# Stalfoes/dqn_mgsc_zoo

Measured on AMD Instinct MI355X. Metric: learner grad-steps/sec at batch=32, 84×84×4 uint8, 1/2/4/8 MI355X, higher is better.
Workload: dtype f32

## Files before the change

dqn_mgsc_zoo_amd/_native.py:

```python

import ctypes
import glob
import hashlib
import os
import threading

_HERE = os.path.dirname(os.path.abspath(__file__))
LIB_PATH = os.environ.get('DQZ_LIB') or os.path.join(_HERE, 'libdqz.so')
HEADER_PATH = os.path.join(os.path.dirname(_HERE), 'include', 'dqz.h')

DQZ_OK = 0
ALGO_DQN = 0
ALGO_DOUBLE = 1
ALGO_PER = 2
NUM_LEAVES = 10
NUM_PHASES = 10
PHASE_NAMES = (
    'conv1_fwd', 'conv2_fwd', 'conv3_fwd', 'fc1_fwd', 'head', 'fc1_dx',
    'conv3_dx+conv2_dx+fc1_dw+conv3_dw+conv2_dw+conv1_dw', 'unused7',
    'unused8', 'update')
FRAME_H = 84
FRAME_W = 84
STACK = 4
FRAME_BYTES = FRAME_H * FRAME_W
# ... 209 lines not shown
        _int, [ctypes.POINTER(DqzLearnerConfig), _int, _vp,
               ctypes.POINTER(_vp)]),
    'dqz_c51_destroy': (_int, [_vp]),
    'dqz_c51_learner': (_int, [_vp, ctypes.POINTER(_vp)]),
    'dqz_c51_step': (
        _int,
        [_vp, ctypes.POINTER(DqzParams), ctypes.POINTER(DqzStore), _vp, _vp,
         _vp, _vp]),
    'dqz_c51_grad': (
        _int,
        [_vp, ctypes.POINTER(DqzParams), ctypes.POINTER(DqzStore), _vp, _vp,
         _vp]),
    'dqz_c51_outputs': (_int, [_vp, _vp, _vp, _vp, _vp, _vp, _vp]),
    'dqz_c51_debug': (_int, [_vp, _vp, _vp, _vp]),
    'dqz_c51_profile': (
        _int,
        [_vp, ctypes.POINTER(DqzParams), ctypes.POINTER(DqzStore), _vp, _vp,
         _int, ctypes.POINTER(ctypes.c_float), _vp]),
    'dqz_c51_forward': (_int, [_vp, _vp, _vp, _int, _vp, _vp]),
    'dqz_c51_forward_slots': (
        _int, [_vp, _vp, ctypes.POINTER(DqzStore), _vp, _int, _int, _vp, _vp]),
    'dqz_c51_act': (
        _int, [_vp, _vp, _vp, _int, ctypes.c_double, ctypes.c_uint64,
               ctypes.c_uint64, _vp, _vp]),
    'dqz_c51_debug_check': (_int, [_int, ctypes.c_uint]),
    'dqz_learner_grad': (
        _int,
        [_vp, ctypes.POINTER(DqzParams), ctypes.POINTER(DqzStore), _vp, _vp,
         _vp, _vp],
    ),
    'dqz_learner_outputs': (_int, [_vp, _vp, _vp, _vp, _vp]),
    'dqz_learner_sync_status': (_int, [_vp, _vp]),
    'dqz_learner_debug_stall': (_int, [_vp, _int, ctypes.c_uint]),
    'dqz_learner_debug_activations': (_int, [_vp, _int] + [_vp] * 10),
    'dqz_per_write_back': (_int, [_vp, _vp, _i64, _vp, ctypes.c_double, _vp, _vp]),
    'dqz_learner_profile': (
        _int,
        [_vp, ctypes.POINTER(DqzParams), ctypes.POINTER(DqzStore), _vp, _vp,
         _int, ctypes.POINTER(ctypes.c_float), _vp],
    ),
    'dqz_forward': (_int, [_vp, _vp, _vp, _int, _vp, _vp]),
    'dqz_forward_slots': (
        _int, [_vp, _vp, ctypes.POINTER(DqzStore), _vp, _int, _int, _vp, _vp]),
    'dqz_act': (
        _int, [_vp, _vp, _vp, _int, ctypes.c_double, ctypes.c_uint64,
               ctypes.c_uint64, _vp, _vp]),
    'dqz_store_put': (
        _int, [ctypes.POINTER(DqzStore), ctypes.POINTER(DqzTransitionPut), _vp,
               _vp]),
    'dqz_store_jumble': (
        _int, [ctypes.POINTER(DqzStore), ctypes.POINTER(DqzJumble), _vp]),
    'dqz_logits_census': (_int, [_vp, _vp, _vp, _i64, _i64, _vp, _vp]),
    'dqz_frame_plan_create': (_int, [_int, _int, _int, _int, ctypes.POINTER(_vp)]),
    'dqz_frame_plan_destroy': (_int, [_vp]),
    'dqz_atari_frame': (_int, [_vp, _vp, _int, _vp, _vp]),
    'dqz_sample_uniform': (
        _int, [_i64, _i64, _i64, _int, ctypes.c_uint64, _vp, _vp, _vp]),
    'dqz_gather_stacks': (
        _int, [ctypes.POINTER(DqzStore), _vp, _int, _int, _vp, _vp]),
    'dqz_target_copy': (_int, [_vp, _vp, _i64, _vp]),
    'dqz_logit_buffer_create': (_int, [_i64, _int, ctypes.POINTER(_vp)]),
    'dqz_logit_buffer_destroy': (_int, [_vp]),
    'dqz_logits_add': (_int, [_vp, _vp, _i64, _i64, _i64, _vp, _vp]),
    'dqz_logits_sample': (_int, [_vp, _vp, _vp, _int, _vp, _vp]),
    'dqz_logits_sample_slots': (
        _int, [_vp, _vp, ctypes.c_uint64, _vp, _vp, _int, _vp, _vp, _vp]),
# ... 130 lines not shown
```

dqn_mgsc_zoo_amd/csrc/bwd.hpp:

```cpp
#pragma once
#include "common.hpp"
#include "conv1.hpp"
#include "fwd.hpp"
#include "head.hpp"
#include "sampling.hpp"

namespace dqz {

struct Fc1BwdArgs {
  const float* dz1;
  const float* y3;
  float *th, *mu, *nu;
  int64_t w_off;
  Rms rms;
  int B;
  float* dy3;
  const float *w3, *w2;
  float *w3p, *w2p;
};

__device__ __forceinline__ int w3p_src(int i) {
  const int j = i & 3, kq = (i >> 2) & 3, n = (i >> 4) & 15, w = (i >> 8) & 3, r = i >> 10;
  const int tp = r % 9, nq = r / 9;
  return ((8 - tp) * C3CI + 16 * nq + n) * C3CO + 16 * w + 4 * j + kq;
// ... 217 lines not shown
    for (int tp = 0; tp < 9; ++tp) {
      const int off = (tp / 3) * C3W_RS + (tp % 3) * C3W_S;
      acc[tp] = mfma4(dr[kk], s_win[pb[kk] + off], acc[tp]);
    }
  float sb = 0.f;
#pragma unroll
  for (int kk = 0; kk < 13; ++kk) sb += dr[kk];
  float* slab = a.part + (int64_t)b * (C3KK + 1) * C3CO;
#pragma unroll
  for (int tp = 0; tp < 9; ++tp)
    *reinterpret_cast<f32x4*>(slab + (tp * C3CI + 16 * w + n) * C3CO + 16 * nq + 4 * kq) = acc[tp];
  if (w == 0) {
    sb += __shfl_xor(sb, 16, 64);
    sb += __shfl_xor(sb, 32, 64);
    if (kq == 0) slab[C3KK * C3CO + 16 * nq + n] = sb;
  }
}

constexpr int C2X_S = 66, C2X_RS = 756, C2X_WIN = 11 * C2X_RS;
constexpr int C2W_S = 40, C2W_RS = 808, C2W_WIN = 20 * C2W_RS;

struct Conv2BwdArgs {
  const float* dy2;
  const float* y1;
  const float* w2;
  const float* w2p;
  float* dy1;
  float* part;
  int B;
  Handoff sync;
  Handoff sync1;
};

template <bool WAIT, bool PUB = false>
__device__ __forceinline__ void conv2_bwd_dx(const Conv2BwdArgs& a, float* s_win, int b, int ph, int pw, int hh) {
  const int t = threadIdx.x, lane = t & 63, w = t >> 6;
  const int n = lane & 15, kq = lane >> 4;
  float wr[16];
  {
    const float4* wp =
        reinterpret_cast<const float4*>(a.w2p) + (((((ph * 2 + pw) * 2 + hh) * 4) * 4 + w) * 16 + n) * 4 + kq;
#pragma unroll
    for (int tp = 0; tp < 4; ++tp) {
      const float4 v = wp[tp * 256];
      wr[4 * tp] = v.x;
      wr[4 * tp + 1] = v.y;
      wr[4 * tp + 2] = v.z;
      wr[4 * tp + 3] = v.w;
    }
  }
  float4 ym4[2];
#pragma unroll
  for (int k = 0; k < 2; ++k) {
    const int q = min((t >> 2) + 64 * k, 99), ah = q / 10, cw = q % 10;
    ym4[k] = *reinterpret_cast<const float4*>(a.y1 + ((int64_t)b * C1M + (2 * ah + ph) * C1O + 2 * cw + pw) * C1CO +
                                              16 * hh + 4 * (t & 3));
  }
  const float4* src = reinterpret_cast<const float4*>(a.dy2 + (int64_t)b * (C2M * C2CO));
  constexpr int NW4 = 121 * 16;
  if constexpr (WAIT) a.sync.wait(b);
  float4 r[8];
#pragma unroll
  for (int q = 0; q < 8; ++q) {
    const int i = min(t + 256 * q, NW4 - 1);
    const int pix = i >> 4, oh = pix / 11 - 1, ow = pix % 11 - 1;
    const bool in = oh >= 0 && oh < C2O && ow >= 0 && ow < C2O;
    const int e = (in ? oh * C2O + ow : 0) * 16 + (i & 15);
    float4 v;
    if constexpr (WAIT)
      v = load_sc1_f4(src, C2M * C2CO * 4, e);
    else
      v = src[e];
    r[q] = in ? v : make_float4(0.f, 0.f, 0.f, 0.f);
  }
  __builtin_amdgcn_sched_barrier(0);
#pragma unroll
  for (int q = 0; q < 8; ++q) {
    const int i = t + 256 * q;
    if (i < NW4) {
      const int pix = i >> 4;
      float* d = s_win + (pix / 11) * C2X_RS + (pix % 11) * C2X_S + win64_ch((i & 15) * 4);
      d[0] = r[q].x;
      d[1] = r[q].y;
      d[2] = r[q].z;
      d[3] = r[q].w;
    }
  }
  __syncthreads();
  DQZ_STAMP(7, 1);
// ... 340 lines not shown
  d += dpp_f<0x140>(d);
  if ((t & 15) == 0) a.dy3[r] = ym > 0.f ? d : 0.f;
  if (a.w3p) {
    if (g < W3P_N) a.w3p[g] = v3;
    if (g < W2P_N) a.w2p[g] = v2;
  }
  DQZ_STAMP(5, 3);
}

#ifdef DQZ_STEP_TU
inline hipError_t launch_head_dx1(const HeadArgs& h, const Fc1BwdArgs& f, hipStream_t st) {
  if (h.S > 7 || h.Z < 1 || h.Z > 3 || h.B != 1) return hipErrorInvalidValue;
  const dim3 grid(FC1X1_BLOCKS), block(512);
  if (h.A <= 8) {
    if (h.Z <= 2)
      hipLaunchKernelGGL((head_dx1_kernel<8, 7, 2>), grid, block, 0, st, h, f);
    else
      hipLaunchKernelGGL((head_dx1_kernel<8, 7, 3>), grid, block, 0, st, h, f);
  } else {
    if (h.Z <= 2)
      hipLaunchKernelGGL((head_dx1_kernel<MAXA, 7, 2>), grid, block, 0, st, h, f);
    else
      hipLaunchKernelGGL((head_dx1_kernel<MAXA, 7, 3>), grid, block, 0, st, h, f);
  }
  return hipGetLastError();
}
#endif

DQZ_STEP_KERNEL __launch_bounds__(256) void fc1_dx_kernel(Fc1BwdArgs a) {
  __shared__ __attribute__((aligned(16))) float smem[FC1X_SMEM];
  fc1_dx_block(a, smem, blockIdx.x);
}

template <bool WB>
__global__ __launch_bounds__(256) __attribute__((amdgpu_waves_per_eu(4, 8))) void bwd_bc_kernel(
    Conv3BwdArgs c3, Fc1BwdArgs f1, Conv2BwdArgs c2, Conv1DwArgs c1, PerWbArgs wb) {
  constexpr int kW = C3X_WIN > FC1W_SMEM ? C3X_WIN : FC1W_SMEM;
  constexpr int kW2 = C2X_WIN > C3W_WIN ? C2X_WIN : C3W_WIN;
  constexpr int kW3 = C2V_WIN > C1H_SMEM ? C2V_WIN : C1H_SMEM;
  constexpr int kWA = kW > kW2 ? kW : kW2;
  constexpr int kSmem = kWA > kW3 ? kWA : kW3;
  static_assert(kSmem * 4 >= PWB_LDS_BYTES, "the write-back's LDS comes out of the backward's buffer");
  __shared__ __attribute__((aligned(16))) float smem[kSmem];
  const int B8 = (c3.B + 7) / 8 * 8;
  constexpr int NF = 4 * (FLAT / 16);
  int i = blockIdx.x;
  if constexpr (WB) {
    if (i < 8) {
      if (i == 0 && threadIdx.x < 64) per_write_back_wave(wb, reinterpret_cast<char*>(smem));
      return;
    }
    i -= 8;
  }
  if (i < 8 * B8) {
    const SampleJob sj = xcd_sample_job_at(i, 8, c3.B);
    if (!sj.valid) return;
    __builtin_amdgcn_s_setprio(3);
    DQZ_STAMP(6, 0);
    conv3_bwd_dx<true>(c3, smem, sj.s, sj.job & 3, sj.job >> 2);
    DQZ_STAMP(6, 3);
    return;
  }
  i -= 8 * B8;
  if (i < NF) {
    fc1_dw_body(f1, smem, i);
    return;
  }
  i -= NF;
  if (i < 8 * B8) {
    const SampleJob sj = xcd_sample_job_at(i, 8, c2.B);
    if (!sj.valid) return;
    __builtin_amdgcn_s_setprio(3);
    DQZ_STAMP(7, 0);
    conv2_bwd_dx<true, true>(c2, smem, sj.s, (sj.job & 3) >> 1, sj.job & 1, sj.job >> 2);
    DQZ_STAMP(7, 3);
    return;
  }
  i -= 8 * B8;
  if (i < 4 * B8) {
    const SampleJob sj = xcd_sample_job_at(i, 4, c3.B);
    if (!sj.valid) return;
    DQZ_STAMP(12, 0);
    conv3_bwd_dw(c3, smem, sj.s, sj.job);
    DQZ_STAMP(12, 3);
    return;
  }
  i -= 4 * B8;
  if (i < 8 * B8) {
    const SampleJob sj = xcd_sample_job_at(i, 8, c1.B);
    if (!sj.valid) return;
    __builtin_amdgcn_s_setprio(2);
    conv1_dw_half(c1, smem, sj.job >> 1, sj.job & 1, sj.s);
    return;
  }
  i -= 8 * B8;
  const SampleJob sj = xcd_sample_job_at(i, 8, c2.B);
  if (!sj.valid) return;
  DQZ_STAMP(13, 0);
  conv2_bwd_dw_split(c2, smem, sj.s, sj.job >> 1, sj.job & 1);
  DQZ_STAMP(13, 3);
}

}
```

dqn_mgsc_zoo_amd/csrc/conv1.hpp:

```cpp
#pragma once
#include "common.hpp"
#include "sampling.hpp"

namespace dqz {

struct Conv1Src {
  const uint8_t* frames;
  const int32_t* fidx;
  const int32_t* slots;
  const uint8_t* states;
  int fused;
  union {
    UniformDraw draw;
    SoftmaxDraw sm;
    PerSampleArgs per;
    SoftmaxDrawExact smx;
  };
  const int32_t* action = nullptr;
  const float* reward = nullptr;
  const float* discount = nullptr;
  float4* rec = nullptr;
  uint8_t* xout = nullptr;
};

// ... 212 lines not shown
    for (int e = 0; e < 4; ++e) {
      const float y = div255(sum[e]) + bb[e];
      v[e] = linear ? y : relu(y);
    }
    if constexpr (PUB) {
      store_sc1_f4(out, C1_POS * C1CO * 4, 16 * i, v);
    } else if (dot) {
      const f32x4 d = *reinterpret_cast<const f32x4*>(dyp + 4 * i);
      dacc += ((v[0] * d[0] + v[1] * d[1]) + (v[2] * d[2] + v[3] * d[3]));
    } else {
      *reinterpret_cast<f32x4*>(out + 4 * i) = v;
    }
  }
  if constexpr (PUB) a.pub.arrive(sj.s);
  if (!PUB && dot) {
    __syncthreads();
    const float r = block_sum256(dacc, smem);
    if (threadIdx.x == 0) a.dot.part[(int64_t)b * META_DOT_SLOTS + a.dot.slot0 + rb] = r;
  }
  DQZ_STAMP(0, 3);
}

struct Conv1DwArgs {
  Conv1Src src;
  int which, B;
  const float* dy1;
  float* part;
  Handoff sync1;
};

constexpr int C1H_TLD = 136;
constexpr int C1H_SMEM = (2 * C1_PLANE * 2 + 3 * C1CO * C1H_TLD * 2) / 4 + 16 * C1CO;

__device__ __forceinline__ void conv1_dw_half(const Conv1DwArgs& a, float* smem, int rb, int ch, int b) {
  DQZ_STAMP(8, 0);
  uint16_t* s_in = reinterpret_cast<uint16_t*>(smem);
  uint16_t* s_dt = s_in + 2 * C1_PLANE;
  float* s_bp = smem + (2 * C1_PLANE + 3 * C1CO * C1H_TLD) / 2;
  const int row0 = rb * C1S * C1_ROWS;
  constexpr int QPC = C1_PLANE / 16;
  const int slot = a.src.slots[b];
  const int32_t* fr = a.src.fidx + (int64_t)slot * 8 + a.which * 4 + 2 * ch;
  const int fa = fr[0], fb = fr[1];
  uint4 v = make_uint4(0u, 0u, 0u, 0u);
  const int tid = threadIdx.x;
  const int cl = tid / QPC, pj = tid % QPC;
  const int f = cl == 0 ? fa : fb;
  if (tid < 2 * QPC && f >= 0)
    v = reinterpret_cast<const uint4*>(a.src.frames + (int64_t)f * FB + row0 * FW)[pj];
  a.sync1.wait(b);
  const float* dyb = a.dy1 + ((int64_t)b * C1M + rb * C1_POS) * C1CO;
  const int co = tid & 31, c0 = tid >> 5;
  float dv[2][8];
#pragma unroll
  for (int it = 0; it < 2; ++it) {
    const int c = c0 + 8 * it, oh = c / 3, ow0 = 8 * (c % 3);
#pragma unroll
    for (int j = 0; j < 8; ++j)
      dv[it][j] = (c < 15 && ow0 + j < C1O)
                      ? load_sc1_f1(dyb, C1_POS * C1CO * 4, (oh * C1O + ow0 + j) * C1CO + co) : 0.f;
  }
  if (tid < 2 * QPC) store_bytes_as_bf16(s_in + cl * C1_PLANE + pj * 16, v);
#pragma unroll
  for (int it = 0; it < 2; ++it) {
    const int c = c0 + 8 * it;
    unsigned pk[3][4];
    float sb = 0.f;
#pragma unroll
    for (int j = 0; j < 8; j += 2) {
      unsigned h0, m0, l0, h1, m1, l1;
      split3_bf16(dv[it][j], h0, m0, l0);
      split3_bf16(dv[it][j + 1], h1, m1, l1);
      pk[0][j / 2] = h0 | (h1 << 16);
      pk[1][j / 2] = m0 | (m1 << 16);
      pk[2][j / 2] = l0 | (l1 << 16);
      sb += dv[it][j];
      sb += dv[it][j + 1];
    }
#pragma unroll
    for (int q = 0; q < 3; ++q)
      *reinterpret_cast<uint4*>(s_dt + (q * C1CO + co) * C1H_TLD + 8 * c) =
          make_uint4(pk[q][0], pk[q][1], pk[q][2], pk[q][3]);
// ... 9 lines not shown
    for (int c = 0; c < 15; ++c) sb += s_bp[c * C1CO + tid];
    part[C1KK * C1CO + tid] = sb;
  }
  const int kh = 2 * wave + (i >> 4), kw = (i >> 1) & 7, cp = i & 1;
  const uint16_t* pb = s_in + cp * C1_PLANE + kh * FW + kw;
  const uint16_t* pa = s_dt + i * C1H_TLD + 8 * h;
  f32x16 acc = {};
#pragma unroll
  for (int s = 0; s < 8; ++s) {
    constexpr int R = 4 * FW;
    const int o0 = (2 * s) / 3 * R + 32 * ((2 * s) % 3);
    const int o1 = 2 * s + 1 < 15 ? (2 * s + 1) / 3 * R + 32 * ((2 * s + 1) % 3) : 0;
    const uint16_t* px = pb + (h ? o1 : o0);
    unsigned xp[4];
#pragma unroll
    for (int j = 0; j < 8; j += 2) xp[j / 2] = (unsigned)px[4 * j] | ((unsigned)px[4 * j + 4] << 16);
    const bf16x8 xb = __builtin_bit_cast(bf16x8, make_uint4(xp[0], xp[1], xp[2], xp[3]));
#pragma unroll
    for (int q = 0; q < 3; ++q) {
      const bf16x8 dq = __builtin_bit_cast(bf16x8, *reinterpret_cast<const uint4*>(pa + q * C1CO * C1H_TLD + 16 * s));
      acc = __builtin_amdgcn_mfma_f32_32x32x16_bf16(dq, xb, acc, 0, 0, 0);
    }
  }
  {
    const int row = (2 * wave + (i >> 4)) * 32 + ((i >> 1) & 7) * 4 + 2 * ch + (i & 1);
#pragma unroll
    for (int q = 0; q < 4; ++q)
      *reinterpret_cast<f32x4*>(part + row * C1CO + 8 * q + 4 * h) =
          f32x4{div255(acc[4 * q]), div255(acc[4 * q + 1]), div255(acc[4 * q + 2]), div255(acc[4 * q + 3])};
  }
  DQZ_STAMP(8, 3);
}

}
```

dqn_mgsc_zoo_amd/csrc/learner_impl.hpp:

```cpp
#pragma once
#include <hip/hip_runtime.h>

#include <cstring>

#include "common.hpp"
#include "layout.hpp"
#include "conv1.hpp"
#include "fwd.hpp"
#include "head.hpp"
#include "bwd.hpp"
#include "sampling.hpp"

namespace dqz {

inline void param_layout(int A, int shared_bias, int64_t off[10], int64_t sz[10], int64_t* total) {
  const int64_t sizes[10] = {C1KK * C1CO, C1CO, C2KK * C2CO, C2CO, C3KK * C3CO, C3CO,
                             (int64_t)FLAT * HID, HID, (int64_t)HID * A, shared_bias ? 1 : A};
  int64_t o = 0;
  for (int i = 0; i < 10; ++i) {
    off[i] = o;
    sz[i] = sizes[i];
    o += (sizes[i] + 63) / 64 * 64;
  }
  *total = o;
}

}

struct dqz_learner {
  dqz_learner_config cfg;
  int Z, shared_bias;
  int64_t off[10], sz[10], total;
  int S_fc1, S2, S3;
  float *y1, *y2, *y3, *fc1p, *h1, *q, *dz1, *dy3, *dy2, *dy1, *p1, *p2, *p3, *td, *loss, *loss_part, *gq, *rec;
  float *w3p, *w2p;
  double* per_wb;
  int32_t* ga;
  int32_t* sync;
  unsigned spin_max = 1u << 24;
  void* block;
};

namespace dqz {

static_assert(Handoff::kStride == kWordStride, "layout.hpp's word stride is Handoff's");

inline SyncLayout sync_of(const dqz_learner* L) { return SyncLayout{L->cfg.batch}; }
inline Handoff handoff(const dqz_learner* L, const HandoffWords& w) {
  Handoff h{L->sync + w.cnt, L->sync + w.ack, L->sync + sync_of(L).err(), w.need, w.consumers};
  if (w.learner_spin) h.spin_max = L->spin_max;
  return h;
}

inline int check_store(const dqz_store* S) {
  if (!S || !S->frames || !S->fidx || !S->action || !S->reward || !S->discount)
    return fail(DQZ_ERR_INVALID, "store has a null buffer");
  if (S->capacity < 1) return fail(DQZ_ERR_INVALID, "store capacity must be positive");
  return DQZ_OK;
}

inline int device_view(const void* p, const void** out, const char* what) {
  hipPointerAttribute_t attr;
  if (hipPointerGetAttributes(&attr, p) != hipSuccess) {
    (void)hipGetLastError();
    return fail(DQZ_ERR_INVALID, "%s must be device memory or pinned host memory", what);
  }
  if (attr.type == hipMemoryTypeHost) {
    void* d = attr.devicePointer;
    if (!d && hipHostGetDevicePointer(&d, const_cast<void*>(p), 0) != hipSuccess) {
      (void)hipGetLastError();
      return fail(DQZ_ERR_INVALID, "%s: pinned host memory without a device mapping", what);
    }
    *out = d;
  } else if (attr.type == hipMemoryTypeDevice || attr.type == hipMemoryTypeManaged ||
             attr.type == hipMemoryTypeUnified) {
    *out = p;
  } else {
    return fail(DQZ_ERR_INVALID, "%s must be device memory or pinned host memory", what);
  }
  return DQZ_OK;
}

struct PhaseEvents {
  hipEvent_t e0, e1;
// ... 109 lines not shown
```

dqn_mgsc_zoo_amd/csrc/learner_step.hip:

```cpp
#define DQZ_STEP_TU 1
#include <hip/hip_runtime.h>

#include <cstdlib>
#include <cstring>

#include "learner_impl.hpp"

using namespace dqz;

static int g_attr_done = 0;

static int init_kernel_attrs() {
  if (g_attr_done) return DQZ_OK;
  const void* fwd_kernels[] = {(const void*)fwd_conv_kernel<0>, (const void*)fwd_conv_kernel<1>,
                               (const void*)fwd_conv_kernel<2>, (const void*)fwd_conv_kernel<3>,
                               (const void*)fwd_conv_kernel<4>};
  for (const void* k : fwd_kernels)
    DQZ_HIP(hipFuncSetAttribute(k, hipFuncAttributeMaxDynamicSharedMemorySize, (int)kConv1FwdSmem));
  g_attr_done = 1;
  return DQZ_OK;
}

extern "C" {

// ... 252 lines not shown
    DQZ_PHASE(4, DQZ_HIP(launch_head(h, B, st)));
    DQZ_PHASE(5, hipLaunchKernelGGL(fc1_dx_kernel, dim3(fc1_dx_blocks(B)), dim3(256), 0, st, fb);
              DQZ_HIP(hipGetLastError()));
  }

  Conv3BwdArgs c3b{};
  c3b.dy3 = L->dy3;
  c3b.y2 = L->y2;
  c3b.w3 = P->online + L->off[4];
  c3b.w3p = L->w3p;
  c3b.dy2 = L->dy2;
  c3b.part = L->p3;
  c3b.B = B;
  c3b.sync = handoff(L, sync_of(L).dy2());
  Conv2BwdArgs c2b{};
  c2b.dy2 = L->dy2;
  c2b.y1 = L->y1;
  c2b.w2 = P->online + L->off[2];
  c2b.w2p = L->w2p;
  c2b.dy1 = L->dy1;
  c2b.part = L->p2;
  c2b.B = B;
  c2b.sync = c3b.sync;
  Conv1DwArgs c1dw{};
  c1dw.src = src;
  c1dw.src.rec = nullptr;
  c1dw.src.xout = nullptr;
  c1dw.which = 0;
  c1dw.B = B;
  c1dw.dy1 = L->dy1;
  c1dw.part = L->p1;
  c1dw.sync1 = handoff(L, sync_of(L).dy1());
  c2b.sync1 = c1dw.sync1;
  const int B8 = (B + 7) / 8 * 8;
  PerWbArgs wbk{};
  const bool wb = r.wb != nullptr;
  if (wb) {
    wbk = *r.wb;
    wbk.td = L->td;
    wbk.n = B;
  }
  const int grid = (wb ? 8 : 0) + 8 * B8 + 4 * (FLAT / 16) + 8 * B8 + 4 * B8 + 8 * B8 + 8 * B8;
  DQZ_PHASE(6, if (wb) hipLaunchKernelGGL(bwd_bc_kernel<true>, dim3(grid), dim3(256), 0, st, c3b, fb, c2b, c1dw, wbk);
            else hipLaunchKernelGGL(bwd_bc_kernel<false>, dim3(grid), dim3(256), 0, st, c3b, fb, c2b, c1dw, wbk);
            DQZ_HIP(hipGetLastError()));
  if (pe.on() && !r.c51) pe.ms[7] = pe.ms[8] = 0.f;

  UpdArgs u{};
  u.th = P->online;
  u.mu = P->mu;
  u.nu = P->nu;
  for (int i = 0; i < 10; ++i) {
    u.off[i] = L->off[i];
    u.sz[i] = L->sz[i];
  }
  u.p1 = L->p1;
  u.p2 = L->p2;
  u.p3 = L->p3;
  u.S1 = B * C1_BLOCKS;
  u.S2 = L->S2;
  u.S3 = L->S3;
  u.h1 = L->h1;
  u.dz1 = L->dz1;
  u.gq = L->gq;
  u.ga = L->ga;
  u.loss_part = L->loss_part;
  u.loss = L->loss;
  u.status = L->sync + sync_of(L).err();
  u.A = r.c51 ? 0 : A;
  u.B = B;
  u.nb2 = r.c51 ? 0 : L->shared_bias ? 1 : A;
  u.rms = rms;
  u.rms.sq_off = 4 * (FLAT / 16);
  const unsigned nblk = update_blocks(L->sz, u.A, u.nb2);
  DQZ_PHASE(9, hipLaunchKernelGGL(update_kernel, dim3(nblk), dim3(256), 0, st, u);
            DQZ_HIP(hipGetLastError()));
  if (r.c51) DQZ_PHASE(7, if (int rc = c51_launch(C51_FC2_GRAD, L, P, r, st)) return rc);
// ... 45 lines not shown
  PhaseEvents pe{nullptr, nullptr, iters, phase_ms};
  DQZ_HIP(hipEventCreate(&pe.e0));
  DQZ_HIP(hipEventCreate(&pe.e1));
  const int rc = step_impl(L, P, S, {.slots = slots, .is_weights = is_weights, .pe = pe}, stream);
  (void)hipEventDestroy(pe.e0);
  (void)hipEventDestroy(pe.e1);
  return rc;
}

int dqz_learner_sync_status(dqz_learner* L, int* status) {
  if (!L || !status) return fail(DQZ_ERR_INVALID, "null argument");
  DQZ_HIP(hipDeviceSynchronize());
  DQZ_HIP(hipMemcpy(status, L->sync + sync_of(L).err(), sizeof(int), hipMemcpyDeviceToHost));
  if (*status != 0) {
    DQZ_HIP(hipMemset(L->sync, 0, sizeof(int) * sync_of(L).ints()));
    DQZ_HIP(hipDeviceSynchronize());
  }
  return DQZ_OK;
}

int dqz_learner_debug_stall(dqz_learner* L, int sample, unsigned spin_max) {
  if (!L) return fail(DQZ_ERR_INVALID, "null learner");
  if (sample >= L->cfg.batch) return fail(DQZ_ERR_INVALID, "sample out of range");
  L->spin_max = spin_max ? spin_max : 1u << 24;
  if (sample >= 0) {
    const int32_t poison = -(1 << 30);
    const SyncLayout at = sync_of(L);
    DQZ_HIP(hipDeviceSynchronize());
    DQZ_HIP(hipMemcpy(L->sync + at.dy2().cnt + at.word(sample), &poison, sizeof(poison), hipMemcpyHostToDevice));
  }
  return DQZ_OK;
}

int dqz_learner_outputs(dqz_learner* L, float* q_tm1, float* td, float* loss, void* stream) {
  if (!L) return fail(DQZ_ERR_INVALID, "null learner");
  hipStream_t st = (hipStream_t)stream;
  const int B = L->cfg.batch, A = L->cfg.num_actions;
  if (q_tm1) DQZ_HIP(hipMemcpyAsync(q_tm1, L->q, sizeof(float) * B * A, hipMemcpyDeviceToDevice, st));
  if (td) DQZ_HIP(hipMemcpyAsync(td, L->td, sizeof(float) * B, hipMemcpyDeviceToDevice, st));
  if (loss) DQZ_HIP(hipMemcpyAsync(loss, L->loss, sizeof(float), hipMemcpyDeviceToDevice, st));
  return DQZ_OK;
}

static int forward_q(dqz_learner* L, const float* params, const Conv1Src& src, int which, int n, float* q_out,
                     hipStream_t st) {
  const NetZ nz{{params, params, params}, {which, which, which}};
  if (int rc = forward_impl(L, nz, 1, n, src, st, PhaseEvents{})) return rc;
  HeadArgs h = make_head(L, nz, 1, n);
  h.fwd_only = 1;
  h.q = q_out;
  DQZ_HIP(launch_head(h, n, st));
  DQZ_HIP(hipGetLastError());
  return DQZ_OK;
}

int dqz_forward(dqz_learner* L, const float* params, const uint8_t* states, int n, float* q_out, void* stream) {
  if (!L || !params || !states || !q_out) return fail(DQZ_ERR_INVALID, "null argument");
  if (n < 1 || n > L->cfg.batch) return fail(DQZ_ERR_INVALID, "n must be in [1, %d]", L->cfg.batch);
  if (reinterpret_cast<uintptr_t>(states) % 16) return fail(DQZ_ERR_INVALID, "states must be 16-byte aligned");
  Conv1Src src{nullptr, nullptr, nullptr, states, 0, UniformDraw{}};
  return forward_q(L, params, src, 0, n, q_out, (hipStream_t)stream);
}

int dqz_forward_slots(dqz_learner* L, const float* params, const dqz_store* S, const int32_t* slots, int n, int which,
                      float* q_out, void* stream) {
  if (!L || !params || !slots || !q_out) return fail(DQZ_ERR_INVALID, "null argument");
// ... 47 lines not shown
```

dqn_mgsc_zoo_amd/learner.py:

```python

import ctypes

import numpy as np
import torch

from dqn_mgsc_zoo_amd import _native
from dqn_mgsc_zoo_amd import networks as networks_lib
from dqn_mgsc_zoo_amd import optim_state

ALGOS = {'dqn': _native.ALGO_DQN, 'double': _native.ALGO_DOUBLE,
         'per': _native.ALGO_PER}


class RMSPropConfig:

  def __init__(self, learning_rate, decay=0.9, eps=1e-8, centered=False):
    self.learning_rate = float(learning_rate)
    self.decay = float(decay)
    self.eps = float(eps)
    self.centered = bool(centered)


def rmsprop(learning_rate, decay=0.9, eps=1e-8, centered=False):
  return RMSPropConfig(learning_rate, decay, eps, centered)
# ... 258 lines not shown
    ms = [float(x) for x in out]
    names = list(_native.PHASE_NAMES)
    return {n: t for n, t in zip(names, ms) if t > 0.0}

  def _need_fused_rmsprop(self, what):
    if self._opt_h is not None:
      raise NotImplementedError(
          '%s runs the fused centered-RMSProp step only; this learner applies '
          '%s after the step (dqz_learner_step_opt*)' % (
              what, type(self.base_optimizer).__name__))

  def grad_norm(self, stream=None):
    if self._opt_h is None:
      raise NotImplementedError(
          'the fused centered-RMSProp step does not keep its gradient; use '
          'Learner.grad()')
    _native.check(_native.lib().dqz_optimizer_outputs(
        self._opt_h, _native.ptr(self._gnorm), _native.stream_handle(stream)))
    return self._gnorm

  def fetch_outputs(self, stream=None):
    _native.check(_native.lib().dqz_learner_outputs(
        self._h, _native.ptr(self.q_tm1), _native.ptr(self.td),
        _native.ptr(self.loss), _native.stream_handle(stream)))
    return self.q_tm1, self.td, self.loss

  def sync_status(self):
    st = ctypes.c_int(0)
    _native.check(_native.lib().dqz_learner_sync_status(self._h, ctypes.byref(st)))
    return st.value

  def debug_stall(self, sample, spin_max=0):
    _native.check(_native.lib().dqz_learner_debug_stall(self._h, int(sample), int(spin_max)))

  def fetch_activations(self, z=0, backward=False, stream=None):
    b, a = self.batch_size, self.network.num_actions
    shapes = dict(y1=(b, 20, 20, 32), y2=(b, 9, 9, 64), y3=(b, 7, 7, 64),
                  h1=(b, 512), q=(b, a))
    if backward:
      shapes.update(dz1=(b, 512), dy3=(b, 7, 7, 64), dy2=(b, 9, 9, 64),
                    dy1=(b, 20, 20, 32))
    out = {k: torch.empty(s, dtype=torch.float32, device=self.device)
           for k, s in shapes.items()}
    _native.check(_native.lib().dqz_learner_debug_activations(
        self._h, int(z),
        *(_native.ptr(out.get(k)) for k in ('y1', 'y2', 'y3', 'h1', 'q', 'dz1',
                                             'dy3', 'dy2', 'dy1')),
        _native.stream_handle(stream)))
    return out

  def q_values(self, states, params=None, stream=None):
    params = self.online if params is None else params
    states = states.contiguous()
    n = int(states.shape[0])
    out = torch.empty((n, self.network.num_actions), dtype=torch.float32,
                      device=self.device)
    for i in range(0, n, self.batch_size):
      j = min(n, i + self.batch_size)
      _native.check(_native.lib().dqz_forward(
          self._h, _native.ptr(params), _native.ptr(states[i:j]), j - i,
          _native.ptr(out[i:j]), _native.stream_handle(stream)))
    return out

  def _params_tensor(self, params):
    if params is None:
      return self.online
# ... 358 lines not shown
```

include/dqz.h:

```cpp
#ifndef DQZ_H_
#define DQZ_H_

#include <stdint.h>

#ifdef __cplusplus
extern "C" {
#endif

#define DQZ_OK 0
#define DQZ_ERR_INVALID (-1)
#define DQZ_ERR_HIP (-2)
#define DQZ_ERR_UNSUPPORTED (-3)

#define DQZ_ALGO_DQN 0
#define DQZ_ALGO_DOUBLE 1
#define DQZ_ALGO_PER 2

#define DQZ_FRAME_H 84
#define DQZ_FRAME_W 84
#define DQZ_STACK 4
#define DQZ_FRAME_BYTES (DQZ_FRAME_H * DQZ_FRAME_W)
#define DQZ_NUM_LEAVES 10

const char* dqz_last_error(void);
// ... 40 lines not shown

int dqz_learner_step_uniform(dqz_learner* learner, const dqz_params* params, const dqz_store* store,
                             int64_t base, int64_t size, int64_t capacity, uint64_t seed,
                             uint64_t* counter_dev, int32_t* slots_out, void* stream);

int dqz_learner_step_per(dqz_learner* learner, const dqz_params* params, const dqz_store* store,
                         const int32_t* slots, const float* is_weights, double* tree, int64_t cap,
                         const int32_t* indices, double alpha, double* max_seen_dev, void* stream);

typedef struct dqz_logit_buffer dqz_logit_buffer;
int dqz_learner_step_logits(dqz_learner* learner, const dqz_params* params, const dqz_store* store,
                            dqz_logit_buffer* buf, const float* logits, uint64_t seed, uint64_t* counter_dev,
                            const double* uniforms, int32_t* slots_out, void* stream);

int dqz_learner_step_logits_exact(dqz_learner* learner, const dqz_params* params, const dqz_store* store,
                                  dqz_logit_buffer* buf, const float* logits, uint64_t seed,
                                  uint64_t* counter_dev, const double* uniforms, int32_t* slots_out,
                                  void* stream);

int dqz_learner_grad(dqz_learner* learner, const dqz_params* params, const dqz_store* store,
                     const int32_t* slots, const float* is_weights, float* grad_out, void* stream);

#define DQZ_NUM_PHASES 10

int dqz_learner_profile(dqz_learner* learner, const dqz_params* params, const dqz_store* store,
                        const int32_t* slots, const float* is_weights, int iters, float* phase_ms,
                        void* stream);

int dqz_learner_outputs(dqz_learner* learner, float* q_tm1, float* td, float* loss, void* stream);

int dqz_learner_sync_status(dqz_learner* learner, int* status);

int dqz_learner_debug_stall(dqz_learner* learner, int sample, unsigned spin_max);

int dqz_learner_debug_activations(dqz_learner* learner, int z, float* y1, float* y2, float* y3, float* h1,
                                  float* q, float* dz1, float* dy3, float* dy2, float* dy1, void* stream);

int dqz_forward(dqz_learner* learner, const float* params, const uint8_t* states, int n,
                float* q_out, void* stream);

int dqz_forward_slots(dqz_learner* learner, const float* params, const dqz_store* store,
                      const int32_t* slots, int n, int which, float* q_out, void* stream);

typedef struct dqz_action {
  int32_t action;
  float value;
} dqz_action;
int dqz_act(dqz_learner* learner, const float* params, const uint8_t* states, int n, double epsilon,
            uint64_t seed, uint64_t counter, dqz_action* out, void* stream);

typedef struct dqz_transition_put {
  int64_t slot;
  int32_t fidx[8];
  int32_t action;
  float reward, discount;
  int32_t num_frames;
  int32_t frame_rows[8];
} dqz_transition_put;
int dqz_store_put(const dqz_store* store, const dqz_transition_put* t, const uint8_t* frames,
                  void* stream);

typedef struct dqz_jumble {
  int64_t slot;
  int64_t src_s_tm1, src_action, src_reward, src_discount, src_s_t;
  int32_t frame_rows[8];
  uint8_t* flags;
// ... 221 lines not shown
```

Measured before the change: 16330.

## Chain conv3 dx, conv2 dx and conv1 dw in one block per sample job

Adds a chained mode to the backward kernel. Each conv3-dx block goes on to run the conv2-dx and conv1-dw work for the same sample and job, and prefetches the weights and frames before waiting on the handoff. This removes 16*B8 separate blocks from the grid and lets the global loads overlap the inter-stage handoff waits. The trade-off is less parallelism across blocks and longer serial chains per block. The mode is on by default for batch sizes 2 to 64, and a debug entry point can toggle it.

New measurement: 16650, median of 6. 1.02x the previous value.

```diff
diff --git a/dqn_mgsc_zoo_amd/_native.py b/dqn_mgsc_zoo_amd/_native.py
--- a/dqn_mgsc_zoo_amd/_native.py
+++ b/dqn_mgsc_zoo_amd/_native.py
@@ -265,6 +265,7 @@
     'dqz_learner_outputs': (_int, [_vp, _vp, _vp, _vp, _vp]),
     'dqz_learner_sync_status': (_int, [_vp, _vp]),
     'dqz_learner_debug_stall': (_int, [_vp, _int, ctypes.c_uint]),
+    'dqz_learner_debug_backward': (_int, [_vp, _int, _vp]),
     'dqz_learner_debug_activations': (_int, [_vp, _int] + [_vp] * 10),
     'dqz_per_write_back': (_int, [_vp, _vp, _i64, _vp, ctypes.c_double, _vp, _vp]),
     'dqz_learner_profile': (
diff --git a/dqn_mgsc_zoo_amd/csrc/bwd.hpp b/dqn_mgsc_zoo_amd/csrc/bwd.hpp
--- a/dqn_mgsc_zoo_amd/csrc/bwd.hpp
+++ b/dqn_mgsc_zoo_amd/csrc/bwd.hpp
@@ -273,11 +273,15 @@
   Handoff sync1;
 };
 
-template <bool WAIT, bool PUB = false>
-__device__ __forceinline__ void conv2_bwd_dx(const Conv2BwdArgs& a, float* s_win, int b, int ph, int pw, int hh) {
+struct Conv2DxOps {
+  float wr[16];
+  float4 ym4[2];
+};
+
+__device__ __forceinline__ void conv2_dx_issue(const Conv2BwdArgs& a, int b, int ph, int pw, int hh, float (&wr)[16],
+                                               float4 (&ym4)[2]) {
   const int t = threadIdx.x, lane = t & 63, w = t >> 6;
   const int n = lane & 15, kq = lane >> 4;
-  float wr[16];
   {
     const float4* wp =
         reinterpret_cast<const float4*>(a.w2p) + (((((ph * 2 + pw) * 2 + hh) * 4) * 4 + w) * 16 + n) * 4 + kq;
@@ -290,12 +294,43 @@
       wr[4 * tp + 3] = v.w;
     }
   }
-  float4 ym4[2];
 #pragma unroll
   for (int k = 0; k < 2; ++k) {
     const int q = min((t >> 2) + 64 * k, 99), ah = q / 10, cw = q % 10;
     ym4[k] = *reinterpret_cast<const float4*>(a.y1 + ((int64_t)b * C1M + (2 * ah + ph) * C1O + 2 * cw + pw) * C1CO +
                                               16 * hh + 4 * (t & 3));
+  }
+}
+
+template <bool WAIT, bool PUB = false, bool PRE = false>
+__device__ __forceinline__ void conv2_bwd_dx(const Conv2BwdArgs& a, float* s_win, int b, int ph, int pw, int hh,
+                                             const Conv2DxOps* pre = nullptr) {
+  const int t = threadIdx.x, lane = t & 63, w = t >> 6;
+  const int n = lane & 15, kq = lane >> 4;
+  float wr[16];
+  float4 ym4[2];
+  if constexpr (PRE) {
+#pragma unroll
+    for (int k = 0; k < 16; ++k) wr[k] = pre->wr[k];
+    ym4[0] = pre->ym4[0];
+    ym4[1] = pre->ym4[1];
+  } else {
+    const float4* wp =
+        reinterpret_cast<const float4*>(a.w2p) + (((((ph * 2 + pw) * 2 + hh) * 4) * 4 + w) * 16 + n) * 4 + kq;
+#pragma unroll
+    for (int tp = 0; tp < 4; ++tp) {
+      const float4 v = wp[tp * 256];
+      wr[4 * tp] = v.x;
+      wr[4 * tp + 1] = v.y;
+      wr[4 * tp + 2] = v.z;
+      wr[4 * tp + 3] = v.w;
+    }
+#pragma unroll
+    for (int k = 0; k < 2; ++k) {
+      const int q = min((t >> 2) + 64 * k, 99), ah = q / 10, cw = q % 10;
+      ym4[k] = *reinterpret_cast<const float4*>(a.y1 + ((int64_t)b * C1M + (2 * ah + ph) * C1O + 2 * cw + pw) * C1CO +
+                                                16 * hh + 4 * (t & 3));
+    }
   }
   const float4* src = reinterpret_cast<const float4*>(a.dy2 + (int64_t)b * (C2M * C2CO));
   constexpr int NW4 = 121 * 16;
@@ -702,7 +737,34 @@
   fc1_dx_block(a, smem, blockIdx.x);
 }
 
-template <bool WB>
+__device__ __forceinline__ void bwd_chain_block(const Conv3BwdArgs& c3, const Conv2BwdArgs& c2, const Conv1DwArgs& c1,
+                                                float* smem, int s, int j) {
+  const int ph = (j & 3) >> 1, pw = j & 1, hh = j >> 2, rb = j >> 1, ch = j & 1;
+  const int slot = c1.src.slots[s];
+  DQZ_STAMP(6, 0);
+  conv3_bwd_dx<true>(c3, smem, s, j & 3, j >> 2);
+  DQZ_STAMP(6, 3);
+  DQZ_STAMP(7, 0);
+  Conv2DxOps o2;
+  conv2_dx_issue(c2, s, ph, pw, hh, o2.wr, o2.ym4);
+  const Conv1DwFrames fr = conv1_dw_frame_ids(c1, ch, slot);
+  __builtin_amdgcn_sched_barrier(0);
+  conv2_bwd_dx<true, true, true>(c2, smem, s, ph, pw, hh, &o2);
+  DQZ_STAMP(7, 3);
+  __builtin_amdgcn_s_setprio(2);
+  DQZ_STAMP(8, 0);
+  const uint4 v = conv1_dw_issue(c1, rb, fr);
+  __builtin_amdgcn_sched_barrier(0);
+  conv1_dw_body<true>(c1, smem, v, rb, ch, s);
+}
+
+constexpr int BWD_CHAIN_MAXB = 64;
+inline int bwd_bc_blocks(int B, bool wb, bool chain) {
+  const int B8 = (B + 7) / 8 * 8;
+  return (wb ? 8 : 0) + 8 * B8 + 4 * (FLAT / 16) + 4 * B8 + 8 * B8 + (chain ? 0 : 16 * B8);
+}
+
+template <bool WB, bool CHAIN>
 __global__ __launch_bounds__(256) __attribute__((amdgpu_waves_per_eu(4, 8))) void bwd_bc_kernel(
     Conv3BwdArgs c3, Fc1BwdArgs f1, Conv2BwdArgs c2, Conv1DwArgs c1, PerWbArgs wb) {
   constexpr int kW = C3X_WIN > FC1W_SMEM ? C3X_WIN : FC1W_SMEM;
@@ -726,9 +788,13 @@
     const SampleJob sj = xcd_sample_job_at(i, 8, c3.B);
     if (!sj.valid) return;
     __builtin_amdgcn_s_setprio(3);
-    DQZ_STAMP(6, 0);
-    conv3_bwd_dx<true>(c3, smem, sj.s, sj.job & 3, sj.job >> 2);
-    DQZ_STAMP(6, 3);
+    if constexpr (CHAIN) {
+      bwd_chain_block(c3, c2, c1, smem, sj.s, sj.job);
+    } else {
+      DQZ_STAMP(6, 0);
+      conv3_bwd_dx<true>(c3, smem, sj.s, sj.job & 3, sj.job >> 2);
+      DQZ_STAMP(6, 3);
+    }
     return;
   }
   i -= 8 * B8;
@@ -737,16 +803,18 @@
     return;
   }
   i -= NF;
-  if (i < 8 * B8) {
-    const SampleJob sj = xcd_sample_job_at(i, 8, c2.B);
-    if (!sj.valid) return;
-    __builtin_amdgcn_s_setprio(3);
-    DQZ_STAMP(7, 0);
-    conv2_bwd_dx<true, true>(c2, smem, sj.s, (sj.job & 3) >> 1, sj.job & 1, sj.job >> 2);
-    DQZ_STAMP(7, 3);
-    return;
-  }
-  i -= 8 * B8;
+  if constexpr (!CHAIN) {
+    if (i < 8 * B8) {
+      const SampleJob sj = xcd_sample_job_at(i, 8, c2.B);
+      if (!sj.valid) return;
+      __builtin_amdgcn_s_setprio(3);
+      DQZ_STAMP(7, 0);
+      conv2_bwd_dx<true, true>(c2, smem, sj.s, (sj.job & 3) >> 1, sj.job & 1, sj.job >> 2);
+      DQZ_STAMP(7, 3);
+      return;
+    }
+    i -= 8 * B8;
+  }
   if (i < 4 * B8) {
     const SampleJob sj = xcd_sample_job_at(i, 4, c3.B);
     if (!sj.valid) return;
@@ -756,14 +824,16 @@
     return;
   }
   i -= 4 * B8;
-  if (i < 8 * B8) {
-    const SampleJob sj = xcd_sample_job_at(i, 8, c1.B);
-    if (!sj.valid) return;
-    __builtin_amdgcn_s_setprio(2);
-    conv1_dw_half(c1, smem, sj.job >> 1, sj.job & 1, sj.s);
-    return;
-  }
-  i -= 8 * B8;
+  if constexpr (!CHAIN) {
+    if (i < 8 * B8) {
+      const SampleJob sj = xcd_sample_job_at(i, 8, c1.B);
+      if (!sj.valid) return;
+      __builtin_amdgcn_s_setprio(2);
+      conv1_dw_half(c1, smem, sj.job >> 1, sj.job & 1, sj.s);
+      return;
+    }
+    i -= 8 * B8;
+  }
   const SampleJob sj = xcd_sample_job_at(i, 8, c2.B);
   if (!sj.valid) return;
   DQZ_STAMP(13, 0);
diff --git a/dqn_mgsc_zoo_amd/csrc/conv1.hpp b/dqn_mgsc_zoo_amd/csrc/conv1.hpp
--- a/dqn_mgsc_zoo_amd/csrc/conv1.hpp
+++ b/dqn_mgsc_zoo_amd/csrc/conv1.hpp
@@ -268,22 +268,48 @@
 constexpr int C1H_TLD = 136;
 constexpr int C1H_SMEM = (2 * C1_PLANE * 2 + 3 * C1CO * C1H_TLD * 2) / 4 + 16 * C1CO;
 
-__device__ __forceinline__ void conv1_dw_half(const Conv1DwArgs& a, float* smem, int rb, int ch, int b) {
-  DQZ_STAMP(8, 0);
+struct Conv1DwFrames {
+  int fa, fb;
+};
+
+__device__ __forceinline__ Conv1DwFrames conv1_dw_frame_ids(const Conv1DwArgs& a, int ch, int slot) {
+  const int32_t* fr = a.src.fidx + (int64_t)slot * 8 + a.which * 4 + 2 * ch;
+  return Conv1DwFrames{fr[0], fr[1]};
+}
+
+__device__ __forceinline__ uint4 conv1_dw_issue(const Conv1DwArgs& a, int rb, const Conv1DwFrames fr) {
+  const int row0 = rb * C1S * C1_ROWS;
+  constexpr int QPC = C1_PLANE / 16;
+  uint4 v = make_uint4(0u, 0u, 0u, 0u);
+  const int tid = threadIdx.x;
+  const int cl = tid / QPC, pj = tid % QPC;
+  const int f = cl == 0 ? fr.fa : fr.fb;
+  if (tid < 2 * QPC && f >= 0)
+    v = reinterpret_cast<const uint4*>(a.src.frames + (int64_t)f * FB + row0 * FW)[pj];
+  return v;
+}
+
+template <bool PRE>
+__device__ __forceinline__ void conv1_dw_body(const Conv1DwArgs& a, float* smem, const uint4 vpre, int rb, int ch,
+                                              int b) {
   uint16_t* s_in = reinterpret_cast<uint16_t*>(smem);
   uint16_t* s_dt = s_in + 2 * C1_PLANE;
   float* s_bp = smem + (2 * C1_PLANE + 3 * C1CO * C1H_TLD) / 2;
   const int row0 = rb * C1S * C1_ROWS;
   constexpr int QPC = C1_PLANE / 16;
-  const int slot = a.src.slots[b];
-  const int32_t* fr = a.src.fidx + (int64_t)slot * 8 + a.which * 4 + 2 * ch;
-  const int fa = fr[0], fb = fr[1];
   uint4 v = make_uint4(0u, 0u, 0u, 0u);
   const int tid = threadIdx.x;
   const int cl = tid / QPC, pj = tid % QPC;
-  const int f = cl == 0 ? fa : fb;
-  if (tid < 2 * QPC && f >= 0)
-    v = reinterpret_cast<const uint4*>(a.src.frames + (int64_t)f * FB + row0 * FW)[pj];
+  if constexpr (PRE) {
+    v = vpre;
+  } else {
+    const int slot = a.src.slots[b];
+    const int32_t* fr = a.src.fidx + (int64_t)slot * 8 + a.which * 4 + 2 * ch;
+    const int fa = fr[0], fb = fr[1];
+    const int f = cl == 0 ? fa : fb;
+    if (tid < 2 * QPC && f >= 0)
+      v = reinterpret_cast<const uint4*>(a.src.frames + (int64_t)f * FB + row0 * FW)[pj];
+  }
   a.sync1.wait(b);
   const float* dyb = a.dy1 + ((int64_t)b * C1M + rb * C1_POS) * C1CO;
   const int co = tid & 31, c0 = tid >> 5;
@@ -359,4 +385,9 @@
   DQZ_STAMP(8, 3);
 }
 
-}
+__device__ __forceinline__ void conv1_dw_half(const Conv1DwArgs& a, float* smem, int rb, int ch, int b) {
+  DQZ_STAMP(8, 0);
+  conv1_dw_body<false>(a, smem, make_uint4(0u, 0u, 0u, 0u), rb, ch, b);
+}
+
+}
diff --git a/dqn_mgsc_zoo_amd/csrc/learner_impl.hpp b/dqn_mgsc_zoo_amd/csrc/learner_impl.hpp
--- a/dqn_mgsc_zoo_amd/csrc/learner_impl.hpp
+++ b/dqn_mgsc_zoo_amd/csrc/learner_impl.hpp
@@ -38,6 +38,7 @@
   int32_t* ga;
   int32_t* sync;
   unsigned spin_max = 1u << 24;
+  int bwd_chain = -1;
   void* block;
 };
 
@@ -50,6 +51,11 @@
   Handoff h{L->sync + w.cnt, L->sync + w.ack, L->sync + sync_of(L).err(), w.need, w.consumers};
   if (w.learner_spin) h.spin_max = L->spin_max;
   return h;
+}
+
+inline bool bwd_chain_active(const dqz_learner* L) {
+  if (L->cfg.batch > BWD_CHAIN_MAXB) return false;
+  return L->bwd_chain < 0 ? L->cfg.batch > 1 : L->bwd_chain != 0;
 }
 
 inline int check_store(const dqz_store* S) {
diff --git a/dqn_mgsc_zoo_amd/csrc/learner_step.hip b/dqn_mgsc_zoo_amd/csrc/learner_step.hip
--- a/dqn_mgsc_zoo_amd/csrc/learner_step.hip
+++ b/dqn_mgsc_zoo_amd/csrc/learner_step.hip
@@ -308,7 +308,6 @@
   c1dw.part = L->p1;
   c1dw.sync1 = handoff(L, sync_of(L).dy1());
   c2b.sync1 = c1dw.sync1;
-  const int B8 = (B + 7) / 8 * 8;
   PerWbArgs wbk{};
   const bool wb = r.wb != nullptr;
   if (wb) {
@@ -316,9 +315,11 @@
     wbk.td = L->td;
     wbk.n = B;
   }
-  const int grid = (wb ? 8 : 0) + 8 * B8 + 4 * (FLAT / 16) + 8 * B8 + 4 * B8 + 8 * B8 + 8 * B8;
-  DQZ_PHASE(6, if (wb) hipLaunchKernelGGL(bwd_bc_kernel<true>, dim3(grid), dim3(256), 0, st, c3b, fb, c2b, c1dw, wbk);
-            else hipLaunchKernelGGL(bwd_bc_kernel<false>, dim3(grid), dim3(256), 0, st, c3b, fb, c2b, c1dw, wbk);
+  const bool chain = bwd_chain_active(L);
+  const dim3 grid(bwd_bc_blocks(B, wb, chain));
+  auto* const bwd = wb ? (chain ? bwd_bc_kernel<true, true> : bwd_bc_kernel<true, false>)
+                       : (chain ? bwd_bc_kernel<false, true> : bwd_bc_kernel<false, false>);
+  DQZ_PHASE(6, hipLaunchKernelGGL(bwd, grid, dim3(256), 0, st, c3b, fb, c2b, c1dw, wbk);
             DQZ_HIP(hipGetLastError()));
   if (pe.on() && !r.c51) pe.ms[7] = pe.ms[8] = 0.f;
 
@@ -430,6 +431,14 @@
   return DQZ_OK;
 }
 
+int dqz_learner_debug_backward(dqz_learner* L, int chain, int* active) {
+  if (!L) return fail(DQZ_ERR_INVALID, "null learner");
+  if (chain < -1 || chain > 1) return fail(DQZ_ERR_INVALID, "chain must be -1, 0 or 1");
+  L->bwd_chain = chain;
+  if (active) *active = bwd_chain_active(L) ? 1 : 0;
+  return DQZ_OK;
+}
+
 int dqz_learner_outputs(dqz_learner* L, float* q_tm1, float* td, float* loss, void* stream) {
   if (!L) return fail(DQZ_ERR_INVALID, "null learner");
   hipStream_t st = (hipStream_t)stream;
diff --git a/dqn_mgsc_zoo_amd/learner.py b/dqn_mgsc_zoo_amd/learner.py
--- a/dqn_mgsc_zoo_amd/learner.py
+++ b/dqn_mgsc_zoo_amd/learner.py
@@ -314,6 +314,12 @@
 
   def debug_stall(self, sample, spin_max=0):
     _native.check(_native.lib().dqz_learner_debug_stall(self._h, int(sample), int(spin_max)))
+
+  def debug_backward(self, chain=-1):
+    active = ctypes.c_int(-1)
+    _native.check(_native.lib().dqz_learner_debug_backward(
+        self._h, int(chain), ctypes.byref(active)))
+    return active.value
 
   def fetch_activations(self, z=0, backward=False, stream=None):
     b, a = self.batch_size, self.network.num_actions
diff --git a/include/dqz.h b/include/dqz.h
--- a/include/dqz.h
+++ b/include/dqz.h
@@ -96,6 +96,8 @@
 int dqz_learner_sync_status(dqz_learner* learner, int* status);
 
 int dqz_learner_debug_stall(dqz_learner* learner, int sample, unsigned spin_max);
+
+int dqz_learner_debug_backward(dqz_learner* learner, int chain, int* active);
 
 int dqz_learner_debug_activations(dqz_learner* learner, int z, float* y1, float* y2, float* y3, float* h1,
                                   float* q, float* dz1, float* dy3, float* dy2, float* dy1, void* stream);
```
